# Hagtaril/HiddenPose

Hardware: AMD Instinct MI355X
Metric: samples/sec (128x128x512 meas) fwd+bwd (higher is better)
Workload: dtype f32; 1 GPU; NlosPose train step (fwd+L2Joint+BCEDice loss+bwd+Adam), 128x128x512 transients, batch 4/GPU, fp32, random-init weights, weight gradients of the 3^3 / 4^3 convolutions (and of small 1^3 ones) on a second stream; global_batch=4, world_size=1, parallelism=dp1

## Files before the change

hiddenpose_amd/csrc/conv_kernels.hip:

```cpp
#include <algorithm>
#include <cstdlib>
#include <cstring>
#include <mutex>
#include <type_traits>
#include <vector>

#include "hp_internal.h"

namespace hp {

using f32x16 = __attribute__((ext_vector_type(16))) float;
using bf16x8 = __attribute__((ext_vector_type(8))) __bf16;
using bf16x4 = __attribute__((ext_vector_type(4))) __bf16;
using bf16x2 = __attribute__((ext_vector_type(2))) __bf16;
using f32x2 = __attribute__((ext_vector_type(2))) float;
using s16x4 = __attribute__((ext_vector_type(4))) short;

__device__ __forceinline__ bf16x4 to_bf16x4(const float4 v) {
  const bf16x2 lo = __builtin_convertvector((f32x2){v.x, v.y}, bf16x2);
  const bf16x2 hi = __builtin_convertvector((f32x2){v.z, v.w}, bf16x2);
  return (bf16x4){lo[0], lo[1], hi[0], hi[1]};
}

enum IgemmMode { MODE_CONV = 0, MODE_DECONV = 1, MODE_DGRAD_S2K3 = 2, MODE_STEM = 3 };
// ... 2016 lines not shown
    for (int i = 0; i < 2; ++i)
#pragma unroll
      for (int r = 0; r < 16; ++r) {
        const int co = i * 32 + (r & 3) + 8 * (r >> 2) + 4 * half;
        if (tap < 343) atomicAdd(dW + (long)co * kpad + tap, acc[i][j][r]);
      }
  }
}

constexpr int SFH_TZ = 16, SFH_TY = 4, SFH_TX = 8, SFH_PZ = SFH_TZ + 6, SFH_PR = 28, SFH_PP = 10 * SFH_PR;
constexpr int SFH_COPY = SFH_PZ * SFH_PP + 8;
constexpr int SFH_W = 50 * 64 * 8;
constexpr int SFH_NP = SFH_PZ * 10 * 14;
constexpr int SFH_LD = (SFH_NP + 511) / 512;

__global__ __launch_bounds__(512) void k_stem_fwd_bf16(const float* __restrict__ X, const float* __restrict__ Wp,
                                                       float* __restrict__ Y, double* __restrict__ stats, int D, int H, int W,
                                                       int kpad, int pz, int py, int px, long tiles_total, int tiles_per_wg) {
  extern __shared__ __attribute__((aligned(16))) float sfh_smem[];
  __bf16* const wl = (__bf16*)sfh_smem;
  __bf16* const patch = wl + SFH_W;
  float* const red = (float*)(patch + 4 * SFH_COPY);
  const int tid = threadIdx.x, lane = tid & 63, wave = tid >> 6, col = lane & 31, half = lane >> 5;
  for (int sidx = tid; sidx < 50 * 64; sidx += 512) {
    const int pr = sidx >> 6, n = sidx & 63;
    float v[8];
#pragma unroll
    for (int c = 0; c < 8; ++c) v[c] = (pr < 49 && c < 7) ? Wp[(long)n * kpad + pr * 7 + c] : 0.f;
    *(bf16x4*)(wl + sidx * 8) = to_bf16x4(make_float4(v[0], v[1], v[2], v[3]));
    *(bf16x4*)(wl + sidx * 8 + 4) = to_bf16x4(make_float4(v[4], v[5], v[6], v[7]));
  }
  for (int i = tid; i < 4 * SFH_COPY / 2; i += 512) ((unsigned int*)patch)[i] = 0u;
  const long t0 = (long)blockIdx.x * tiles_per_wg, t1 = min(tiles_total, t0 + tiles_per_wg);
  float preg[SFH_LD];
  auto tile_origin = [&](long t, int& b, int& z0, int& y0, int& x0) {
    long r_ = t;
    x0 = (int)(r_ % px) * SFH_TX;
    r_ /= px;
    y0 = (int)(r_ % py) * SFH_TY;
    r_ /= py;
    z0 = (int)(r_ % pz) * SFH_TZ;
    b = (int)(r_ / pz);
  };
  auto fetch = [&](long t) {
    int b, z0, y0, x0;
    tile_origin(t, b, z0, y0, x0);
#pragma unroll
    for (int k = 0; k < SFH_LD; ++k) {
      const int e = tid + 512 * k;
      const int pzz = e / 140, rem = e - pzz * 140, pyy = rem / 14, pxx = rem - pyy * 14;
      const int z = z0 + pzz - 3, y = y0 + pyy - 3, x = x0 + pxx - 3;
      preg[k] = (e < SFH_NP && (unsigned)z < (unsigned)D && (unsigned)y < (unsigned)H && (unsigned)x < (unsigned)W)
                    ? X[(((long)b * D + z) * H + y) * W + x]
                    : 0.f;
    }
  };
  int abase[2];
#pragma unroll
  for (int mt = 0; mt < 2; ++mt) abase[mt] = (2 * wave + mt) * SFH_PP + (col >> 3) * SFH_PR + (col & 7);
  float ssum[2] = {0.f, 0.f}, ssq[2] = {0.f, 0.f};
  if (t0 < t1) fetch(t0);
  for (long t = t0; t < t1; ++t) {
    __syncthreads();
#pragma unroll
    for (int k = 0; k < SFH_LD; ++k) {
      const int e = tid + 512 * k;
      const int pzz = e / 140, rem = e - pzz * 140, pyy = rem / 14, pxx = rem - pyy * 14;
      if (e < SFH_NP) {
        const int pi = pzz * SFH_PP + pyy * SFH_PR + pxx;
        const __bf16 v = (__bf16)preg[k];
#pragma unroll
        for (int sft = 0; sft < 4; ++sft)
          if (pi - sft >= 0) patch[sft * SFH_COPY + pi - sft] = v;
      }
    }
    __syncthreads();
    int b, z0, y0, x0;
    tile_origin(t, b, z0, y0, x0);
    if (t + 1 < t1) fetch(t + 1);
    f32x16 acc[2][2];
#pragma unroll
    for (int mt = 0; mt < 2; ++mt)
#pragma unroll
      for (int nt = 0; nt < 2; ++nt)
#pragma unroll
        for (int r = 0; r < 16; ++r) acc[mt][nt][r] = 0.f;
    int kd = 0, kh = half;
#pragma unroll 5
    for (int ks = 0; ks < 25; ++ks) {
      const int pr = 2 * ks + half;
      const int off = pr < 49 ? kd * SFH_PP + kh * SFH_PR : 0;
      bf16x8 ha[2], hb[2];
#pragma unroll
      for (int mt = 0; mt < 2; ++mt) {
        const int e = abase[mt] + off;
        const __bf16* const src = patch + (e & 3) * SFH_COPY + (e & ~3);
        union {
          uint2 q[2];
          bf16x8 f;
        } u;
        u.q[0] = *(const uint2*)(src);
        u.q[1] = *(const uint2*)(src + 4);
        ha[mt] = u.f;
      }
#pragma unroll
      for (int nt = 0; nt < 2; ++nt) hb[nt] = *(const bf16x8*)(wl + ((pr * 64) + nt * 32 + col) * 8);
#pragma unroll
      for (int mt = 0; mt < 2; ++mt)
#pragma unroll
        for (int nt = 0; nt < 2; ++nt) acc[mt][nt] = __builtin_amdgcn_mfma_f32_32x32x16_bf16(ha[mt], hb[nt], acc[mt][nt], 0, 0, 0);
      kh += 2;
      if (kh >= 7) {
        kh -= 7;
        ++kd;
      }
    }
#pragma unroll
    for (int mt = 0; mt < 2; ++mt) {
      const int z = z0 + 2 * wave + mt;
#pragma unroll
      for (int r = 0; r < 16; ++r) {
        const int i = (r & 3) + 8 * (r >> 2) + 4 * half;
        const int y = y0 + (i >> 3), x = x0 + (i & 7);
        if (z < D && y < H && x < W) {
          float* const yo = Y + ((((long)b * D + z) * H + y) * W + x) * 64 + col;
#pragma unroll
          for (int nt = 0; nt < 2; ++nt) {
            const float v = acc[mt][nt][r];
            yo[nt * 32] = v;
            ssum[nt] += v;
            ssq[nt] += v * v;
          }
        }
      }
    }
  }
  if (stats) {
#pragma unroll
    for (int nt = 0; nt < 2; ++nt) {
      const float sv = ssum[nt] + __shfl_xor(ssum[nt], 32), qv = ssq[nt] + __shfl_xor(ssq[nt], 32);
      if (half == 0) {
        red[(wave * 64 + nt * 32 + col) * 2 + 0] = sv;
        red[(wave * 64 + nt * 32 + col) * 2 + 1] = qv;
      }
    }
    __syncthreads();
    if (tid < 64) {
      double sv = 0.0, qv = 0.0;
#pragma unroll
      for (int w = 0; w < 8; ++w) {
        sv += (double)red[(w * 64 + tid) * 2 + 0];
        qv += (double)red[(w * 64 + tid) * 2 + 1];
      }
      double* const slot = stats + (size_t)(blockIdx.x & (HP_STATS_SLOTS - 1)) * 128;
      atomicAdd(slot + tid, sv);
      atomicAdd(slot + 64 + tid, qv);
    }
  }
}

constexpr int SF_TY = 8, SF_TX = 64, SF_RY = SF_TY + 6, SF_RX = 72, SF_PLANE = SF_RY * SF_RX;
using f32x4c = __attribute__((ext_vector_type(4))) float;

__global__ __launch_bounds__(256) void k_stem_fwd_mfma(const float* __restrict__ X, const float* __restrict__ Wp,
                                                       float* __restrict__ Y, double* __restrict__ stats, int D, int H, int W,
                                                       int kpad, int tiles_x, int tiles_y, int zchunk) {
  extern __shared__ __attribute__((aligned(16))) float sf_smem[];
  float* const wl = sf_smem;
  float* const ring = wl + 343 * 64;
  float* const otile = ring + 8 * SF_PLANE;
  const int tid = threadIdx.x, lane = tid & 63, wave = tid >> 6, sub = lane & 3;
  int t_ = blockIdx.x;
  const int bx = t_ % tiles_x;
  t_ /= tiles_x;
  const int by = t_ % tiles_y;
  const int bz = t_ / tiles_y;
  const int b = blockIdx.y;
  const int x0 = bx * SF_TX, y0 = by * SF_TY;
  const int zb = bz * zchunk, ze = min(D, zb + zchunk);
  const float* xb = X + (long)b * D * H * W;

  for (int e = tid; e < 343 * 64; e += 256) {
    const int cg = e & 15, i = (e >> 4) & 3, tap = e >> 6;
    wl[e] = Wp[(long)(cg * 4 + i) * kpad + tap];
  }
  constexpr int SK = (SF_PLANE + 255) / 256;
  int soff[SK];
  unsigned smask = 0;
#pragma unroll
  for (int k = 0; k < SK; ++k) {
    const int e = tid + 256 * k;
    const int ly = e / SF_RX, lx = e - ly * SF_RX;
    const int yy = y0 + ly - 3, xx = x0 + lx - 3;
    const bool ok = e < SF_PLANE && lx < SF_TX + 6 && (unsigned)yy < (unsigned)H && (unsigned)xx < (unsigned)W;
    soff[k] = ok ? yy * W + xx : 0;
    smask |= ok ? (1u << k) : 0u;
  }
  auto stage_load = [&](int zin, float (&v)[SK]) {
    const bool zok = (unsigned)zin < (unsigned)D;
    const float* src = xb + (long)(zok ? zin : 0) * H * W;
#pragma unroll
    for (int k = 0; k < SK; ++k) v[k] = (zok && ((smask >> k) & 1u)) ? src[soff[k]] : 0.f;
  };
  auto stage_store = [&](int zin, const float (&v)[SK]) {
    float* dst = ring + (zin & 7) * SF_PLANE + tid;
#pragma unroll
    for (int k = 0; k < SK; ++k)
      if (tid + 256 * k < SF_PLANE) dst[256 * k] = v[k];
  };
  auto stage = [&](int zin) {
    float v[SK];
    stage_load(zin, v);
    stage_store(zin, v);
  };
  if (zb < ze)
    for (int zin = zb - 3; zin <= zb + 3; ++zin) stage(zin);
  __syncthreads();

  float* const ot = otile + wave * (64 * 33);
  float ssum[2] = {0.f, 0.f}, ssq[2] = {0.f, 0.f};
  for (int z = zb; z < ze; ++z) {
    float nv[SK];
    if (z + 1 < ze) stage_load(z + 4, nv);
    __builtin_amdgcn_sched_barrier(0);
    f32x4c acc[2][16];
#pragma unroll
    for (int r = 0; r < 2; ++r)
#pragma unroll
      for (int cg = 0; cg < 16; ++cg) acc[r][cg] = (f32x4c){0.f, 0.f, 0.f, 0.f};
#pragma unroll 1
    for (int a = 0; a < 7; ++a) {
      const float* pl = ring + ((z + a - 3) & 7) * SF_PLANE + (2 * wave) * SF_RX + lane;
#pragma unroll
      for (int bb = 0; bb < 7; ++bb) {
        const float* wt = wl + ((a * 7 + bb) * 7) * 64 + sub * 16;
#pragma unroll
        for (int c = 0; c < 7; ++c) {
          float wr[16];
#pragma unroll
          for (int q = 0; q < 4; ++q) {
            const f32x4c t4 = *(const f32x4c*)(wt + c * 64 + 4 * q);
            wr[4 * q] = t4[0];
            wr[4 * q + 1] = t4[1];
            wr[4 * q + 2] = t4[2];
            wr[4 * q + 3] = t4[3];
          }
#pragma unroll
          for (int r = 0; r < 2; ++r) {
            const float xv = pl[(r + bb) * SF_RX + c];
#pragma unroll
            for (int cg = 0; cg < 16; ++cg) acc[r][cg] = __builtin_amdgcn_mfma_f32_4x4x1f32(wr[cg], xv, acc[r][cg], 0, 0, 0);
          }
        }
      }
    }
#pragma unroll
    for (int r = 0; r < 2; ++r) {
      const int oy = y0 + 2 * wave + r;
      const bool row_ok = oy < H;
      const long orow = (((long)b * D + z) * H + oy) * W + x0;
#pragma unroll
      for (int hh = 0; hh < 2; ++hh) {
#pragma unroll
        for (int cg = 0; cg < 8; ++cg)
#pragma unroll
          for (int i = 0; i < 4; ++i) ot[lane * 33 + cg * 4 + i] = acc[r][8 * hh + cg][i];
        if (row_ok) {
          if (stats && lane < 32) {
            float s = 0.f, q = 0.f;
            const int nv = min(64, W - x0);
            for (int v = 0; v < nv; ++v) {
              const float val = ot[v * 33 + lane];
              s += val;
              q += val * val;
            }
            ssum[hh] += s;
            ssq[hh] += q;
          }
          const int q4 = lane & 7;
#pragma unroll
          for (int it = 0; it < 8; ++it) {
            const int v = it * 8 + (lane >> 3);
            if (x0 + v < W) {
              const float* sp = ot + v * 33 + 4 * q4;
              *(float4*)(Y + (orow + v) * 64 + 32 * hh + 4 * q4) = make_float4(sp[0], sp[1], sp[2], sp[3]);
            }
          }
        }
      }
    }
    if (z + 1 < ze) stage_store(z + 4, nv);
    __syncthreads();
  }
  if (stats && lane < 32) {
#pragma unroll
    for (int hh = 0; hh < 2; ++hh) {
      double* const slot = stats + (size_t)(blockIdx.x & (HP_STATS_SLOTS - 1)) * 128;
      atomicAdd(slot + 32 * hh + lane, (double)ssum[hh]);
      atomicAdd(slot + 64 + 32 * hh + lane, (double)ssq[hh]);
    }
  }
}

__global__ void k_pack_weight(const float* __restrict__ w, float* __restrict__ out, int Cout, int Cin, int taps,
                              int transposed, int swap, int to_torch) {
  const long total = (long)Cout * Cin * taps;
  for (long i = (long)blockIdx.x * blockDim.x + threadIdx.x; i < total; i += (long)gridDim.x * blockDim.x) {
    const int inner = (int)(i % (swap ? Cout : Cin));
    long r = i / (swap ? Cout : Cin);
    const int outer = (int)(r % (swap ? Cin : Cout));
    const int t = (int)(r / (swap ? Cin : Cout));
    const int co = swap ? inner : outer, ci = swap ? outer : inner;
    const long ti = transposed ? ((long)ci * Cout + co) * taps + t : ((long)co * Cin + ci) * taps + t;
    if (to_torch)
      ((float*)w)[ti] = out[i];
    else
      out[i] = w[ti];
  }
}

__global__ __launch_bounds__(256) void k_pack_weight_tiled(const float* __restrict__ w, float* __restrict__ out, int Cout,
                                                           int Cin, int taps, int transposed, int swap, int to_torch,
                                                           int out_half = 0) {
  __shared__ float tile[64][65];
  const int A = swap ? Cin : Cout, Bn = swap ? Cout : Cin;
  const int a = blockIdx.y, bn0 = blockIdx.x * 64;
  const int nb = min(64, Bn - bn0), n = nb * taps;
  auto torch_index = [&](int bn, int t) -> long {
    const int co = swap ? bn : a, ci = swap ? a : bn;
    return transposed ? ((long)ci * Cout + co) * taps + t : ((long)co * Cin + ci) * taps + t;
  };
  if (!to_torch) {
    for (int e = threadIdx.x; e < n; e += 256) {
      const int bl = e / taps, t = e - bl * taps;
      tile[bl][t] = w[torch_index(bn0 + bl, t)];
    }
    __syncthreads();
    for (int e = threadIdx.x; e < taps * 64; e += 256) {
      const int t = e >> 6, bl = e & 63;
      if (bl < nb) hp_st1(out, ((long)t * A + a) * Bn + bn0 + bl, tile[bl][t], out_half);
    }
  } else {
    for (int e = threadIdx.x; e < taps * 64; e += 256) {
      const int t = e >> 6, bl = e & 63;
      if (bl < nb) tile[bl][t] = out[((long)t * A + a) * Bn + bn0 + bl];
    }
    __syncthreads();
    for (int e = threadIdx.x; e < n; e += 256) {
      const int bl = e / taps, t = e - bl * taps;
      ((float*)w)[torch_index(bn0 + bl, t)] = tile[bl][t];
    }
  }
}

__global__ void k_pack_stem(const float* __restrict__ w, float* __restrict__ out, int Cout, int kpad, int to_torch) {
  const long total = (long)Cout * kpad;
  for (long i = (long)blockIdx.x * blockDim.x + threadIdx.x; i < total; i += (long)gridDim.x * blockDim.x) {
    const int k = (int)(i % kpad), n = (int)(i / kpad);
    if (to_torch) {
      if (k < 343) ((float*)w)[(long)n * 343 + k] = out[i];
    } else {
      out[i] = k < 343 ? w[(long)n * 343 + k] : 0.f;
    }
  }
}

struct ConvPlan {
  IgemmGeom fwd, dgrad, wgrad;
  int fwd_classes = 1, dgrad_classes = 1, wgrad_tapsum = 1;
  bool stem = false, dgrad_zero_fill = false;
  int planes = 0;
};

static void set_shifts(IgemmGeom& g) {
  g.sw = g.sh = g.sd = -1;
  if (g.mode >= 0 && is_pow2(g.gw) && is_pow2(g.gh) && is_pow2(g.gd) && g.M < (1l << 32)) {
    g.sw = ilog2(g.gw);
    g.sh = ilog2(g.gh);
    g.sd = ilog2(g.gd);
  }
}

static int make_plan(const hp_conv_desc& d, ConvPlan& p) {
  HP_REQUIRE(d.B >= 1 && d.Cin >= 1 && d.Cout >= 1, "conv: bad channel/batch sizes");
  HP_REQUIRE(d.precision >= HP_PRECISION_FP32 && d.precision <= HP_PRECISION_BF16X6, "conv: unknown precision %d", d.precision);
  HP_REQUIRE(d.io == 0 || d.precision == HP_PRECISION_BF16, "conv: bf16 activation tensors (io = %d) go with HP_PRECISION_BF16", d.io);
  p.planes = d.precision;
  const int k = d.k, s = d.stride, pad = d.pad;
  IgemmGeom f{};
  if (!d.transposed) {
    const int Do = (d.Di + 2 * pad - k) / s + 1, Ho = (d.Hi + 2 * pad - k) / s + 1, Wo = (d.Wi + 2 * pad - k) / s + 1;
    p.stem = (d.Cin == 1 && k == 7 && s == 1 && pad == 3);
    if (!p.stem) HP_REQUIRE(d.Cin % 4 == 0, "conv: Cin must be a multiple of 4 (got %d)", d.Cin);
    HP_REQUIRE(s == 1 || s == 2, "conv: stride must be 1 or 2");
    const int kpt = p.stem ? (343 + 31) / 32 : (d.Cin + 31) / 32;
    f = IgemmGeom{p.stem ? MODE_STEM : MODE_CONV, d.B, d.Di, d.Hi, d.Wi, d.Cin, Do, Ho, Wo, d.Cout, Do, Ho, Wo, 1,
                  k, s, pad, 0, (long)d.B * Do * Ho * Wo, kpt};
    p.fwd = f;
    p.fwd_classes = 1;
    p.wgrad = f;
    p.wgrad_tapsum = p.stem ? 1 : k * k * k;
    IgemmGeom g{};
    if (p.stem) {
      g = IgemmGeom{MODE_CONV, d.B, Do, Ho, Wo, d.Cout, d.Di, d.Hi, d.Wi, 1, d.Di, d.Hi, d.Wi, 1,
                    7, 1, 3, 1, (long)d.B * d.Di * d.Hi * d.Wi, d.Cout / 32};
      p.dgrad_classes = 1;
    } else if (s == 1) {
      HP_REQUIRE(d.Cout % 4 == 0, "conv dgrad: Cout must be a multiple of 4 (got %d)", d.Cout);
      g = IgemmGeom{MODE_CONV, d.B, Do, Ho, Wo, d.Cout, d.Di, d.Hi, d.Wi, d.Cin, d.Di, d.Hi, d.Wi, 1,
                    k, 1, pad, 1, (long)d.B * d.Di * d.Hi * d.Wi, (d.Cout + 31) / 32};
      p.dgrad_classes = 1;
    } else if (k == 3 && pad == 1) {
      HP_REQUIRE(d.Di % 2 == 0 && d.Hi % 2 == 0 && d.Wi % 2 == 0 && d.Cout % 32 == 0, "conv dgrad s2: even dims needed");
      g = IgemmGeom{MODE_DGRAD_S2K3, d.B, Do, Ho, Wo, d.Cout, d.Di, d.Hi, d.Wi, d.Cin, d.Di / 2, d.Hi / 2, d.Wi / 2, 2,
                    3, 1, 1, 0, (long)d.B * (d.Di / 2) * (d.Hi / 2) * (d.Wi / 2), d.Cout / 32};
      p.dgrad_classes = 8;
    } else if (k == 1 && pad == 0) {
      HP_REQUIRE(d.Di % 2 == 0 && d.Hi % 2 == 0 && d.Wi % 2 == 0 && d.Cout % 32 == 0, "conv dgrad s2: even dims needed");
      g = IgemmGeom{MODE_CONV, d.B, Do, Ho, Wo, d.Cout, d.Di, d.Hi, d.Wi, d.Cin, Do, Ho, Wo, 2,
                    1, 1, 0, 0, (long)d.B * Do * Ho * Wo, d.Cout / 32};
      p.dgrad_classes = 1;
      p.dgrad_zero_fill = true;
    } else {
      set_error("conv: unsupported stride-2 kernel %d pad %d", k, pad);
      return HP_ERR_UNSUPPORTED;
    }
    p.dgrad = g;
  } else {
    HP_REQUIRE(k == 4 && s == 2 && pad == 1, "deconv: only k4 s2 p1 is supported");
    HP_REQUIRE(d.Cin % 32 == 0 && d.Cout % 32 == 0, "deconv: channels must be multiples of 32");
    const int Do = 2 * d.Di, Ho = 2 * d.Hi, Wo = 2 * d.Wi;
    f = IgemmGeom{MODE_DECONV, d.B, d.Di, d.Hi, d.Wi, d.Cin, Do, Ho, Wo, d.Cout, d.Di, d.Hi, d.Wi, 2,
                  4, 1, 1, 0, (long)d.B * d.Di * d.Hi * d.Wi, d.Cin / 32};
    p.fwd = f;
    p.fwd_classes = 8;
    p.wgrad = f;
    p.wgrad_tapsum = 64;
    p.dgrad = IgemmGeom{MODE_CONV, d.B, Do, Ho, Wo, d.Cout, d.Di, d.Hi, d.Wi, d.Cin, d.Di, d.Hi, d.Wi, 1,
                        4, 2, 1, 0, (long)d.B * d.Di * d.Hi * d.Wi, d.Cout / 32};
    p.dgrad_classes = 1;
  }
  HP_REQUIRE((long)d.B * d.Di * d.Hi * d.Wi * (d.transposed ? 8 : 1) < (1l << 31), "conv: more than 2^31 voxels per tensor");
  set_shifts(p.fwd);
  set_shifts(p.dgrad);
  set_shifts(p.wgrad);
  p.fwd.welems = p.wgrad.welems = p.stem ? (long)d.Cout * ((343 + 31) / 32 * 32) : (long)d.Cout * d.Cin * k * k * k;
  p.dgrad.welems = (long)d.Cout * d.Cin * k * k * k;
  return HP_OK;
}

template <bool STEM, bool STATS, int NP, bool XH = false>
static void launch_igemm_bn(const IgemmGeom& g, int classes, const void* X, const float* W, const float* bias, void* Y,
                            double* stats, const void* addend, const unsigned char* amask, hipStream_t st) {
  if constexpr (NP == 1 && !STEM && !XH) {
    if (g.xh && g.Cin % 64 == 0) return launch_igemm_bn<STEM, STATS, NP, true>(g, classes, X, W, bias, Y, stats, addend, amask, st);
  }
  const unsigned mt = (unsigned)((g.M + BM - 1) / BM);
  static const bool gl_on = !(getenv("HP_IGEMM_GL") && atoi(getenv("HP_IGEMM_GL")) == 0);
  const bool gl = XH && g.wh && gl_on;
  static const bool bl_on = !(getenv("HP_IGEMM_BL") && atoi(getenv("HP_IGEMM_BL")) == 0);
  const bool bl = !XH && !g.xh && !g.wh && !STEM && bl_on && g.Cin % 32 == 0 && (long)g.Nout * g.Cin * class_ntaps(g, 0) * 4 * (g.mode == MODE_DECONV ? 8 : 1) < (1l << 31);
  static const bool slab_on = !(getenv("HP_IGEMM_SLAB") && atoi(getenv("HP_IGEMM_SLAB")) == 0);
  if (slab_on && g.Nout <= 64) {
    IgemmGeom gs = g;
    gs.slab = (int)((mt + 7) / 8);
    const dim3 grid((mt + 7) / 8 * 8, 1, classes);
    if constexpr (!XH && !STEM) {
      if (bl && g.Nout > 32) {
        hipLaunchKernelGGL((k_igemm<64, false, STATS, NP, false, false, true>), grid, dim3(CT), 0, st, X, W, bias, Y, stats, addend, amask, gs);
        return;
      }
    }
  }
  if (g.Nout > 64) {
    const unsigned tn = (unsigned)((g.Nout + 127) / 128);
    IgemmGeom gg = g;
    gg.tn = tn > 1 ? (int)tn : 0;
    gg.slab = slab_on ? (int)((mt + 7) / 8) : 0;
    const dim3 grid = (tn > 1 || gg.slab) ? dim3((mt + 7) / 8 * 8 * (tn > 1 ? tn : 1), 1, classes) : dim3(mt, 1, classes);
    if constexpr (XH) {
      if (gl) {
        hipLaunchKernelGGL((k_igemm<128, STEM, STATS, NP, true, true>), grid, dim3(CT), 0, st, X, W, bias, Y, stats, addend, amask, gg);
        return;
      }
    }
    if constexpr (!XH && !STEM) {
      if (bl) {
        hipLaunchKernelGGL((k_igemm<128, false, STATS, NP, false, false, true>), grid, dim3(CT), 0, st, X, W, bias, Y, stats, addend, amask, gg);
        return;
      }
    }
    hipLaunchKernelGGL((k_igemm<128, STEM, STATS, NP, XH>), grid, dim3(CT), 0, st, X, W, bias, Y, stats, addend, amask, gg);
  } else if (g.Nout > 32) {
    if constexpr (XH) {
      if (gl) {
        hipLaunchKernelGGL((k_igemm<64, STEM, STATS, NP, true, true>), dim3(mt, 1, classes), dim3(CT), 0, st, X, W, bias, Y, stats, addend, amask, g);
        return;
      }
    }
    if constexpr (!XH && !STEM) {
      if (bl) {
        hipLaunchKernelGGL((k_igemm<64, false, STATS, NP, false, false, true>), dim3(mt, 1, classes), dim3(CT), 0, st, X, W, bias, Y, stats, addend, amask, g);
        return;
      }
    }
    hipLaunchKernelGGL((k_igemm<64, STEM, STATS, NP, XH>), dim3(mt, 1, classes), dim3(CT), 0, st, X, W, bias, Y, stats, addend, amask, g);
  } else {
    hipLaunchKernelGGL((k_igemm<32, STEM, STATS, NP, XH>), dim3(mt, 1, classes), dim3(CT), 0, st, X, W, bias, Y, stats, addend, amask, g);
  }
}

template <int NP>
static void launch_igemm_p(const IgemmGeom& g, int classes, bool stem, const void* X, const float* W, const float* bias,
                           void* Y, double* stats, const void* addend, const unsigned char* amask, hipStream_t st) {
  if (stem) {
    if (stats) launch_igemm_bn<true, true, NP>(g, classes, X, W, bias, Y, stats, addend, amask, st);
    else launch_igemm_bn<true, false, NP>(g, classes, X, W, bias, Y, stats, addend, amask, st);
  } else {
    if (stats) launch_igemm_bn<false, true, NP>(g, classes, X, W, bias, Y, stats, addend, amask, st);
    else launch_igemm_bn<false, false, NP>(g, classes, X, W, bias, Y, stats, addend, amask, st);
  }
}

static void launch_igemm(const IgemmGeom& g, int classes, bool stem, int planes, const void* X, const float* W,
                         const float* bias, void* Y, double* stats, const void* addend, hipStream_t st,
                         const unsigned char* amask = nullptr) {
  switch (planes) {
    case 1: launch_igemm_p<1>(g, classes, stem, X, W, bias, Y, stats, addend, amask, st); break;
    case 2: launch_igemm_p<2>(g, classes, stem, X, W, bias, Y, stats, addend, amask, st); break;
    case 3: launch_igemm_p<3>(g, classes, stem, X, W, bias, Y, stats, addend, amask, st); break;
    default: launch_igemm_p<0>(g, classes, stem, X, W, bias, Y, stats, addend, amask, st); break;
  }
}

}

using namespace hp;

extern "C" size_t hp_conv3d_packed_weight_elems(const hp_conv_desc* d) {
  if (!d) return 0;
  if (!d->transposed && d->Cin == 1 && d->k == 7) return (size_t)d->Cout * ((343 + 31) / 32 * 32);
  return (size_t)d->Cout * d->Cin * d->k * d->k * d->k;
}

extern "C" int hp_conv3d_pack_weight(const hp_conv_desc* d, const float* w_torch, void* w_fwd_v, void* w_dgrad_v,
                                     void* stream) {
  float* const w_fwd = (float*)w_fwd_v;
  float* const w_dgrad = (float*)w_dgrad_v;
  HP_REQUIRE(d && w_torch, "hp_conv3d_pack_weight: null argument");
  ConvPlan p;
  int rc = make_plan(*d, p);
  if (rc) return rc;
  hipStream_t st = (hipStream_t)stream;
  const int taps = d->k * d->k * d->k;
  if (p.stem) {
    const int kpad = p.fwd.kpt * BK;
    HP_PROF("conv_pack_weight", st);
    if (w_fwd) hipLaunchKernelGGL(k_pack_stem, dim3(64), dim3(256), 0, st, w_torch, w_fwd, d->Cout, kpad, 0);
    if (w_dgrad) hipLaunchKernelGGL(k_pack_weight, dim3(64), dim3(256), 0, st, w_torch, w_dgrad, d->Cout, 1, 343, 0, 1, 0);
  } else {
    HP_REQUIRE(taps <= 64, "conv: at most 64 taps (got %d)", taps);
    HP_PROF("conv_pack_weight", st);
    const int wh = (d->io & HP_IO_W_BF16) ? 1 : 0;
    if (w_fwd)
      hipLaunchKernelGGL(k_pack_weight_tiled, dim3((d->Cin + 63) / 64, d->Cout), dim3(256), 0, st, w_torch, w_fwd, d->Cout,
                         d->Cin, taps, d->transposed, 0, 0, wh);
    if (w_dgrad)
      hipLaunchKernelGGL(k_pack_weight_tiled, dim3((d->Cout + 63) / 64, d->Cin), dim3(256), 0, st, w_torch, w_dgrad, d->Cout,
                         d->Cin, taps, d->transposed, 1, 0, wh);
  }
  HP_CHECK_HIP(hipGetLastError());
  return HP_OK;
}

extern "C" int hp_conv3d_unpack_wgrad(const hp_conv_desc* d, const float* dw_packed, float* dw_torch, void* stream) {
  HP_REQUIRE(d && dw_packed && dw_torch, "hp_conv3d_unpack_wgrad: null argument");
  ConvPlan p;
  int rc = make_plan(*d, p);
  if (rc) return rc;
  hipStream_t st = (hipStream_t)stream;
  const int taps = d->k * d->k * d->k;
  HP_PROF("conv_pack_weight", st);
  if (p.stem) {
    hipLaunchKernelGGL(k_pack_stem, dim3(64), dim3(256), 0, st, dw_torch, (float*)dw_packed, d->Cout, p.fwd.kpt * BK, 1);
  } else {
    hipLaunchKernelGGL(k_pack_weight_tiled, dim3((d->Cin + 63) / 64, d->Cout), dim3(256), 0, st, dw_torch, (float*)dw_packed,
                       d->Cout, d->Cin, taps, d->transposed, 0, 1);
  }
  HP_CHECK_HIP(hipGetLastError());
  return HP_OK;
}

extern "C" int hp_conv3d_forward(const hp_conv_desc* d, const void* x, const float* w_fwd, const float* bias, void* y,
                                 double* stats, void* stream) {
  HP_REQUIRE(d && x && w_fwd && y, "hp_conv3d_forward: null argument");
  ConvPlan p;
  int rc = make_plan(*d, p);
  if (rc) return rc;
  HP_REQUIRE(!(p.stem && (d->io & HP_IO_X_BF16)), "hp_conv3d_forward: the stem reads its single-channel input as fp32");
  p.fwd.xh = (d->io & HP_IO_X_BF16) ? 1 : 0;
  p.fwd.yh = (d->io & HP_IO_Y_BF16) ? 1 : 0;
  p.fwd.wh = (d->io & HP_IO_W_BF16) ? 1 : 0;
  HP_REQUIRE(!p.fwd.wh || (p.fwd.xh && p.planes == 1 && !p.stem && d->Cin % 64 == 0),
             "hp_conv3d_forward: bf16 packed weights go with a bf16 input, HP_PRECISION_BF16 and Cin %% 64 == 0");
  hipStream_t st = (hipStream_t)stream;
  if (stats) HP_CHECK_HIP(hipMemsetAsync(stats, 0, sizeof(double) * 2 * d->Cout * HP_STATS_SLOTS, st));
  if (p.stem && p.planes == 1 && d->Cout == 64 && !bias && !p.fwd.yh) {
    const int pz = (d->Di + SFH_TZ - 1) / SFH_TZ, py = (d->Hi + SFH_TY - 1) / SFH_TY, px = (d->Wi + SFH_TX - 1) / SFH_TX;
    const long tiles = (long)d->B * pz * py * px;
    const int per_wg = (int)std::max<long>(1, (tiles + 511) / 512);
    const size_t lds = sizeof(__bf16) * (SFH_W + 4 * SFH_COPY) + sizeof(float) * 8 * 64 * 2;
    static std::once_flag lds_once_h;
    static hipError_t lds_rc_h = hipSuccess;
    std::call_once(lds_once_h, [&] {
      lds_rc_h = hipFuncSetAttribute((const void*)k_stem_fwd_bf16, hipFuncAttributeMaxDynamicSharedMemorySize, (int)lds);
    });
    HP_CHECK_HIP(lds_rc_h);
    HP_PROF("conv_igemm_stem", st);
    hipLaunchKernelGGL(k_stem_fwd_bf16, dim3((unsigned)((tiles + per_wg - 1) / per_wg)), dim3(512), lds, st, (const float*)x, w_fwd,
                       (float*)y, stats, d->Di, d->Hi, d->Wi, p.fwd.kpt * BK, pz, py, px, tiles, per_wg);
  } else if (p.stem && p.planes == 0 && d->Cout == 64 && !bias && !p.fwd.yh) {
    const int tiles_x = (d->Wi + SF_TX - 1) / SF_TX, tiles_y = (d->Hi + SF_TY - 1) / SF_TY;
    const long cols = (long)tiles_x * tiles_y * d->B;
    int zsplit = (int)std::max<long>(1, std::min<long>((d->Di + 15) / 16, (1024 + cols - 1) / cols));
    const int zchunk = (d->Di + zsplit - 1) / zsplit;
    zsplit = (d->Di + zchunk - 1) / zchunk;
    const size_t lds = sizeof(float) * (343 * 64 + 8 * SF_PLANE + 4 * 64 * 33);
    static std::once_flag lds_once;
    static hipError_t lds_rc = hipSuccess;
    std::call_once(lds_once, [&] {
      lds_rc = hipFuncSetAttribute((const void*)k_stem_fwd_mfma, hipFuncAttributeMaxDynamicSharedMemorySize, (int)lds);
    });
    HP_CHECK_HIP(lds_rc);
    HP_PROF("conv_igemm_stem", st);
    hipLaunchKernelGGL(k_stem_fwd_mfma, dim3((unsigned)(tiles_x * tiles_y * zsplit), (unsigned)d->B), dim3(256), lds, st,
                       (const float*)x, w_fwd, (float*)y, stats, d->Di, d->Hi, d->Wi, p.fwd.kpt * BK, tiles_x, tiles_y, zchunk);
  } else {
    HP_PROF(p.stem ? "conv_igemm_stem" : d->transposed ? "conv_igemm_deconv" : d->k == 1 ? "conv_igemm_k1" : "conv_igemm_k3", st);
    launch_igemm(p.fwd, p.fwd_classes, p.stem, p.planes, x, w_fwd, bias, y, stats, nullptr, st);
  }
  HP_CHECK_HIP(hipGetLastError());
  return HP_OK;
}

extern "C" int hp_linear_forward(const float* x, const float* w, const float* bias, const float* addend, float* y, long M, int K,
                                 int N, int precision, void* stream) {
  HP_REQUIRE(x && w && y && M >= 1 && M < (1l << 31) && K >= 4 && N >= 1, "hp_linear_forward: bad argument");
  hp_conv_desc d{1, 1, 1, (int)M, K, N, 1, 1, 0, 0, precision, 0};
  ConvPlan p;
  int rc = make_plan(d, p);
  if (rc) return rc;
  hipStream_t st = (hipStream_t)stream;
  {
    HP_PROF("linear_fwd", st);
    launch_igemm(p.fwd, 1, false, p.planes, x, w, bias, y, nullptr, addend, st);
  }
  HP_CHECK_HIP(hipGetLastError());
  return HP_OK;
}

extern "C" int hp_linear_geglu_forward(const float* x, const float* w, const float* bias, float* y, long M, int K,
                                       int N2, int precision, void* stream) {
  HP_REQUIRE(x && w && y && M >= 1 && M < (1l << 31) && K >= 4, "hp_linear_geglu_forward: bad argument");
  HP_REQUIRE(N2 >= 128 && N2 % 128 == 0, "hp_linear_geglu_forward: 2 * hidden must be a multiple of 128 (got %d)", N2);
  hp_conv_desc d{1, 1, 1, (int)M, K, N2, 1, 1, 0, 0, precision, 0};
  ConvPlan p;
  int rc = make_plan(d, p);
  if (rc) return rc;
  p.fwd.geglu = 1;
  hipStream_t st = (hipStream_t)stream;
  {
    HP_PROF("linear_fwd", st);
    launch_igemm(p.fwd, 1, false, p.planes, x, w, bias, y, nullptr, nullptr, st);
  }
  HP_CHECK_HIP(hipGetLastError());
  return HP_OK;
}

static bool launch_igemm_bns(const IgemmGeom& g, const void* X, const float* W, void* Y, const void* addend,
                             const unsigned char* amask, hipStream_t st) {
  const bool dense_out = g.os == 1 && g.gd == g.Do && g.gh == g.Ho && g.gw == g.Wo;
  if (g.mode != MODE_CONV || !dense_out || g.M % BM != 0 || g.Nout <= 32 || g.Nout % (g.Nout > 64 ? 128 : 64) != 0 || g.xh || g.yh ||
      g.wh || g.ah)
    return false;
  const unsigned mt = (unsigned)(g.M / BM);
  static const bool bl_on = !(getenv("HP_IGEMM_BL") && atoi(getenv("HP_IGEMM_BL")) == 0);
  static const bool slab_on = !(getenv("HP_IGEMM_SLAB") && atoi(getenv("HP_IGEMM_SLAB")) == 0);
  const bool bl = bl_on && g.Cin % 32 == 0 && (long)g.Nout * g.Cin * class_ntaps(g, 0) * 4 < (1l << 31);
  IgemmGeom gg = g;
  gg.slab = slab_on ? (int)((mt + 7) / 8) : 0;
#define HP_BNS_LAUNCH(BN_, BL_)                                                                                                     \
  do {                                                                                                                             \
    if (g.bn_mask)                                                                                                                 \
      hipLaunchKernelGGL((k_igemm<BN_, false, false, 0, false, false, BL_, 2>), grid, dim3(CT), 0, st, X, W, nullptr, Y, nullptr,   \
                         addend, amask, gg);                                                                                       \
    else                                                                                                                           \
      hipLaunchKernelGGL((k_igemm<BN_, false, false, 0, false, false, BL_, 1>), grid, dim3(CT), 0, st, X, W, nullptr, Y, nullptr,   \
                         addend, amask, gg);                                                                                       \
  } while (0)
  if (g.Nout <= 64) {
    const dim3 grid = gg.slab ? dim3((mt + 7) / 8 * 8, 1, 1) : dim3(mt, 1, 1);
    if (bl) HP_BNS_LAUNCH(64, true);
    else HP_BNS_LAUNCH(64, false);
    return true;
  }
  const unsigned tn = (unsigned)(g.Nout / 128);
  gg.tn = tn > 1 ? (int)tn : 0;
  const dim3 grid = (tn > 1 || gg.slab) ? dim3((mt + 7) / 8 * 8 * (tn > 1 ? tn : 1), 1, 1) : dim3(mt, 1, 1);
  if (bl) HP_BNS_LAUNCH(128, true);
  else HP_BNS_LAUNCH(128, false);
#undef HP_BNS_LAUNCH
  return true;
}

extern "C" int hp_conv3d_backward_data_bnsums(const hp_conv_desc* d, const void* dy, const float* w_dgrad, void* dx, const void* addend,
                                              const unsigned char* addend_mask, const float* z, const float* mean,
                                              const float* rstd, const float* gamma, const float* beta, int relu,
                                              const unsigned char* relu_mask, double* sums, int* fused, void* stream) {
  HP_REQUIRE(d && dy && w_dgrad && dx && z && mean && rstd && sums && fused && (!relu || relu_mask || (gamma && beta)),
             "hp_conv3d_backward_data_bnsums: null argument");
  *fused = 0;
  ConvPlan p;
  int rc = make_plan(*d, p);
  if (rc) return rc;
  hipStream_t st = (hipStream_t)stream;
  if (p.planes == 0 && !p.stem && !p.dgrad_zero_fill && d->io == 0 && p.dgrad_classes == 1 &&
      (!addend_mask || (addend && d->Cin % 4 == 0 && d->Cin > 32))) {
    IgemmGeom g = p.dgrad;
    g.bn_z = z;
    g.bn_mean = mean;
    g.bn_rstd = rstd;
    g.bn_gamma = gamma;
    g.bn_beta = beta;
    g.bn_sums = sums;
    g.bn_relu = relu ? 1 : 0;
    g.bn_mask = relu ? relu_mask : nullptr;
    HP_CHECK_HIP(hipMemsetAsync(sums, 0, sizeof(double) * 2 * g.Nout * HP_STATS_SLOTS, st));
    HP_PROF("conv_igemm_dgrad", st);
    if (launch_igemm_bns(g, dy, w_dgrad, dx, addend, addend_mask, st)) {
      HP_CHECK_HIP(hipGetLastError());
      *fused = 1;
      return HP_OK;
    }
  }
  return hp_conv3d_backward_data_masked(d, dy, w_dgrad, dx, addend, addend_mask, stream);
}

extern "C" int hp_conv3d_backward_data(const hp_conv_desc* d, const void* dy, const float* w_dgrad, void* dx,
                                       const void* addend, void* stream) {
  return hp_conv3d_backward_data_masked(d, dy, w_dgrad, dx, addend, nullptr, stream);
}

extern "C" int hp_conv3d_backward_data_masked(const hp_conv_desc* d, const void* dy, const float* w_dgrad, void* dx,
                                              const void* addend, const unsigned char* addend_mask, void* stream) {
  HP_REQUIRE(d && dy && w_dgrad && dx, "hp_conv3d_backward_data: null argument");
  ConvPlan p;
  int rc = make_plan(*d, p);
  if (rc) return rc;
  const int dyh = (d->io & HP_IO_DY_BF16) ? 1 : 0, dxh = (d->io & HP_IO_DX_BF16) ? 1 : 0;
  HP_REQUIRE(!(p.stem && (dyh || dxh)), "hp_conv3d_backward_data: the stem's data gradient is fp32 in, fp32 out");
  p.dgrad.xh = dyh;
  p.dgrad.yh = p.dgrad.ah = dxh;
  p.dgrad.wh = (d->io & HP_IO_W_BF16) ? 1 : 0;
  HP_REQUIRE(!p.dgrad.wh || (dyh && p.planes == 1 && !p.stem && p.dgrad.Cin % 64 == 0),
             "hp_conv3d_backward_data: bf16 packed weights go with a bf16 dy, HP_PRECISION_BF16 and Cout %% 64 == 0");
  const size_t esz = dxh ? 2 : 4;
  HP_REQUIRE(!addend_mask || (addend && !p.stem && !p.dgrad_zero_fill && d->Cin % 4 == 0 && d->Cin > 32),
             "hp_conv3d_backward_data_masked: a masked addend needs a dense data gradient with > 32 input channels, a multiple of 4");
  hipStream_t st = (hipStream_t)stream;
  if (p.stem) {
    HP_REQUIRE(d->Cout == 64, "stem data gradient: 64 output channels expected (got %d)", d->Cout);
    HP_REQUIRE((long)d->Hi * d->Wi <= (1l << 21), "stem data gradient: H * W up to 2^21 (31-bit offsets inside a 4-plane dZ tile), got %d x %d", d->Hi, d->Wi);
    const size_t nb = sizeof(float) * (size_t)d->B * d->Di * d->Hi * d->Wi;
    if (addend) HP_CHECK_HIP(hipMemcpyAsync(dx, addend, nb, hipMemcpyDeviceToDevice, st));
    else HP_CHECK_HIP(hipMemsetAsync(dx, 0, nb, st));
    const int pz = (d->Di + SP_Z - 1) / SP_Z, py = (d->Hi + SP_Y - 1) / SP_Y, px = (d->Wi + SP_X - 1) / SP_X;
    HP_PROF("conv_stem_dgrad", st);
    const long cols = (long)py * px * d->B;
    int zsplit = 1;
    long best = -1;
    for (int zs = 1; zs <= std::min(pz, 32); ++zs) {
      const long cost = ((cols * zs + 767) / 768) * ((pz + zs - 1) / zs + 2);
      if (best < 0 || cost < best) best = cost, zsplit = zs;
    }
    if (const char* e = getenv("HP_STEM_DGRAD_ZSPLIT")) zsplit = std::max(1, std::min(pz, atoi(e)));
    const int zchunk = (pz + zsplit - 1) / zsplit;
    zsplit = (pz + zchunk - 1) / zchunk;
    hipLaunchKernelGGL(p.planes == 1 ? k_stem_dgrad<true> : k_stem_dgrad<false>, dim3((unsigned)(py * px * zsplit), (unsigned)d->B), dim3(CT), 0,
                       st, (const float*)dy, w_dgrad, (float*)dx, d->Di, d->Hi, d->Wi, pz, py, px, zchunk);
    HP_CHECK_HIP(hipGetLastError());
    return HP_OK;
  }
  if (p.dgrad_zero_fill) {
    const size_t nb = esz * (size_t)d->B * d->Di * d->Hi * d->Wi * d->Cin;
    if (addend == dx) {}
    else if (addend) HP_CHECK_HIP(hipMemcpyAsync(dx, addend, nb, hipMemcpyDeviceToDevice, st));
    else HP_CHECK_HIP(hipMemsetAsync(dx, 0, nb, st));
  }
  {
    HP_PROF("conv_igemm_dgrad", st);
    launch_igemm(p.dgrad, p.dgrad_classes, false, p.planes, dy, w_dgrad, nullptr, dx, nullptr, addend, st, addend_mask);
  }
  HP_CHECK_HIP(hipGetLastError());
  return HP_OK;
}

struct WgradSplit {
  int TT, tap_groups, tiles_c, tiles_total;
  bool multitap;
  long msplit;
};
static WgradSplit wgrad_split(const ConvPlan& p) {
  const IgemmGeom& g = p.wgrad;
  const int Kc = p.stem ? g.kpt * BK : g.Cin;
  WgradSplit w{};
  w.TT = (g.Nout >= 128 && Kc >= 128) ? 128 : 64;
  w.multitap = !p.stem && w.TT == 64 && g.mode == MODE_CONV && g.k == 3;
  w.tap_groups = w.multitap ? (27 + 3) / 4 : p.wgrad_tapsum;
  const int tiles_n = (g.Nout + w.TT - 1) / w.TT;
  w.tiles_c = (Kc + w.TT - 1) / w.TT;
  const long base_blocks = (long)tiles_n * w.tiles_c * w.tap_groups;
  long hi = std::max<long>(1, (4096 + base_blocks - 1) / base_blocks);
  hi = std::min<long>(std::min<long>(hi, std::max<long>(1, g.M / (4 * WG_KM))), 4096);
  static const int fixed_env = getenv("HP_WGRAD_R0") ? atoi(getenv("HP_WGRAD_R0")) : -1;
  const long r0 = fixed_env >= 0 ? fixed_env : ((g.xh && g.yh) ? 768 : 96);
  long best = hi;
  struct Memo { long M, base, r0, hi, best; };
  static std::mutex memo_mu;
  static std::vector<Memo> memo;
  bool known = false;
  {
    std::lock_guard<std::mutex> lk(memo_mu);
    for (const Memo& m : memo)
      if (m.M == g.M && m.base == base_blocks && m.r0 == r0 && m.hi == hi) {
        best = m.best;
        known = true;
        break;
      }
  }
  if (r0 > 0 && !known) {
    const long slots = 768;
    auto cost = [&](long ms) {
      const long rows = ((g.M + ms - 1) / ms + WG_KM - 1) / WG_KM * WG_KM;
      const long blocks = base_blocks * ms;
      double c = (double)((blocks + slots - 1) / slots) * (double)(rows + r0);
      if (blocks & 7) c *= 1.02;
      return c;
    };
    double cmin = cost(hi);
    for (long ms = 1; ms < hi; ++ms) cmin = std::min(cmin, cost(ms));
    for (long ms = hi; ms >= 1; --ms)
      if (cost(ms) <= 1.03 * cmin) {
        best = ms;
        break;
      }
  }
  for (; !known;) {
    const long chunk = ((g.M + best - 1) / best + WG_KM - 1) / WG_KM * WG_KM;
    const long need = (g.M + chunk - 1) / chunk;
    if (need >= best) break;
    best = need;
  }
  if (!known) {
    std::lock_guard<std::mutex> lk(memo_mu);
    if (memo.size() < 4096) memo.push_back({g.M, base_blocks, r0, hi, best});
  }
  w.msplit = best;
  w.tiles_total = tiles_n * w.tiles_c;
  return w;
}

extern "C" int hp_conv3d_backward_weight_split(const hp_conv_desc* d, long* msplit, long* chunk_rows) {
  HP_REQUIRE(d && msplit && chunk_rows, "hp_conv3d_backward_weight_split: null argument");
  ConvPlan p;
  int rc = make_plan(*d, p);
  if (rc) return rc;
  p.wgrad.xh = (d->io & HP_IO_X_BF16) ? 1 : 0;
  p.wgrad.yh = (d->io & HP_IO_DY_BF16) ? 1 : 0;
  const WgradSplit ws = wgrad_split(p);
  *msplit = ws.msplit;
  *chunk_rows = ((p.wgrad.M + ws.msplit - 1) / ws.msplit + WG_KM - 1) / WG_KM * WG_KM;
  return HP_OK;
}

extern "C" int hp_conv3d_backward_weight(const hp_conv_desc* d, const void* x, const void* dy, float* dw_packed,
                                         void* stream) {
  HP_REQUIRE(d && x && dy && dw_packed, "hp_conv3d_backward_weight: null argument");
  ConvPlan p;
  int rc = make_plan(*d, p);
  if (rc) return rc;
  hipStream_t st = (hipStream_t)stream;
  const int xh = (d->io & HP_IO_X_BF16) ? 1 : 0, dyh = (d->io & HP_IO_DY_BF16) ? 1 : 0;
  HP_REQUIRE(!(p.stem && xh), "hp_conv3d_backward_weight: the stem reads its single-channel input as fp32");
  p.wgrad.xh = xh;
  p.wgrad.yh = dyh;
  const IgemmGeom& g = p.wgrad;
  const int Kc = p.stem ? g.kpt * BK : g.Cin;
  HP_CHECK_HIP(hipMemsetAsync(dw_packed, 0, sizeof(float) * hp_conv3d_packed_weight_elems(d), st));
  if (p.stem && p.planes <= 1 && d->Cout == 64 && !dyh) {
    const int pz = (d->Di + SP_Z - 1) / SP_Z, py = (d->Hi + SP_Y - 1) / SP_Y, px = (d->Wi + SP_X - 1) / SP_X;
    const long tiles = (long)d->B * pz * py * px;
    const int per_wg = (int)std::max<long>(1, (tiles + 1023) / 1024);
    HP_PROF("conv_wgrad", st);
    hipLaunchKernelGGL(p.planes == 1 ? k_stem_wgrad_bf16 : k_stem_wgrad_full, dim3((unsigned)((tiles + per_wg - 1) / per_wg)), dim3(256),
                       0, st, (const float*)x, (const float*)dy, dw_packed, d->Di,
                       d->Hi, d->Wi, pz, py, px, tiles, per_wg, Kc);
    HP_CHECK_HIP(hipGetLastError());
    return HP_OK;
  }
  if (!p.stem && p.planes == 0 && !xh && !dyh && g.mode == MODE_CONV && g.k == 1 && g.s == 1 && g.os == 1 && g.M >= (1l << 16)) {
    const bool wide_n = g.Nout % 256 == 0 && g.Cin == 64, wide_c = g.Nout == 64 && g.Cin % 256 == 0;
    if (wide_n || wide_c) {
      const int tiles = wide_n ? g.Nout / 256 : g.Cin / 256;
      long ms = std::max<long>(1, std::min<long>(1024 / tiles, g.M / (4 * WG_KM)));
      ms = std::max<long>(8, ms / 8 * 8);
      HP_PROF("conv_wgrad", st);
      if (wide_n)
        hipLaunchKernelGGL((k_wgrad_dense<256, 64>), dim3((unsigned)(tiles * ms)), dim3(CT), 0, st, (const float*)x, (const float*)dy, dw_packed, g.M, g.Nout,
                           g.Cin, (int)ms, 1);
      else
        hipLaunchKernelGGL((k_wgrad_dense<64, 256>), dim3((unsigned)(tiles * ms)), dim3(CT), 0, st, (const float*)x, (const float*)dy, dw_packed, g.M, g.Nout,
                           g.Cin, (int)ms, tiles);
      HP_CHECK_HIP(hipGetLastError());
      return HP_OK;
    }
  }
  const WgradSplit ws = wgrad_split(p);
  const int TT = ws.TT, tap_groups = ws.tap_groups, tiles_c = ws.tiles_c, tiles_total = ws.tiles_total;
  const bool multitap = ws.multitap;
  const long msplit = ws.msplit;
  dim3 grid((unsigned)((long)tiles_total * tap_groups * msplit));
  {
    HP_PROF("conv_wgrad", st);
    static const bool wbl_on = !(getenv("HP_WGRAD_BL") && atoi(getenv("HP_WGRAD_BL")) == 0);
    const long chunk_rows = (g.M + msplit - 1) / msplit + WG_KM;
    const long span_y = chunk_rows * g.os * g.os * g.os * (long)g.Nout * 4, span_x = (chunk_rows * g.s * g.s * g.s + 4l * g.Hi * g.Wi) * (long)g.Cin * 4;
    const bool exact_grid = g.Di == g.gd * g.s && g.Hi == g.gh * g.s && g.Wi == g.gw * g.s && g.Do == g.gd * g.os &&
                            g.Ho == g.gh * g.os && g.Wo == g.gw * g.os;
    if (wbl_on && !p.stem && p.planes == 0 && !xh && !dyh && g.sw >= 0 && exact_grid && g.Nout % 4 == 0 && g.Cin % 4 == 0 &&
// ... 70 lines not shown
```

Before: 8.783 samples/s.

## Add fp32 stem forward kernel using 32x32x2 MFMA with explicit LDS pipelining

Adds a new stem convolution forward kernel (7^3 taps, Cin=1, Cout=64) built on mfma_f32_32x32x2f32 in place of the older 4x4x1-based route. It pairs taps per MFMA step, issues LDS reads through inline asm with immediate offsets, and double-buffers fragments under explicit waitcnt and sched barriers. BN statistics are reduced in LDS before one atomic per channel. The old kernel stays reachable through an environment variable. This costs extra LDS and register pressure and depends on hand-written asm ordering.

```diff
diff --git a/hiddenpose_amd/csrc/conv_kernels.hip b/hiddenpose_amd/csrc/conv_kernels.hip
--- a/hiddenpose_amd/csrc/conv_kernels.hip
+++ b/hiddenpose_amd/csrc/conv_kernels.hip
@@ -2342,6 +2342,196 @@
   }
 }
 
+constexpr int SF32_WL = 344 * 64;
+constexpr int SF32_ZP = 160;
+
+__device__ __forceinline__ unsigned lds_addr(const float* p) {
+  return (unsigned)(size_t)(const __attribute__((address_space(3))) float*)p;
+}
+
+template <int S, int N, class F>
+__device__ __forceinline__ void static_for(F&& f) {
+  if constexpr (S < N) {
+    f(std::integral_constant<int, S>{});
+    static_for<S + 1, N>(f);
+  }
+}
+
+__global__ __launch_bounds__(256) void k_stem_fwd_mfma32(const float* __restrict__ X, const float* __restrict__ Wp,
+                                                         float* __restrict__ Y, double* __restrict__ stats, int D, int H, int W,
+                                                         int kpad, int tiles_x, int tiles_y, int zchunk) {
+  extern __shared__ __attribute__((aligned(16))) float sf_smem[];
+  float* const wl = sf_smem;
+  float* const ring = wl + SF32_WL;
+  float* const red = ring + 8 * SF_PLANE;
+  float* const zpad = red + 8 * 128;
+  const int tid = threadIdx.x, lane = tid & 63, wave = tid >> 6, col = lane & 31, half = lane >> 5;
+  int t_ = blockIdx.x;
+  const int bx = t_ % tiles_x;
+  t_ /= tiles_x;
+  const int by = t_ % tiles_y;
+  const int bz = t_ / tiles_y;
+  const int b = blockIdx.y;
+  const int x0 = bx * SF_TX, y0 = by * SF_TY;
+  const int zb = bz * zchunk, ze = min(D, zb + zchunk);
+  const float* xb = X + (long)b * D * H * W;
+
+  for (int e = tid; e < SF32_WL; e += 256) {
+    const int n = e & 63, tap = e >> 6;
+    wl[e] = tap < 343 ? Wp[(long)n * kpad + tap] : 0.f;
+  }
+  if (tid < SF32_ZP) zpad[tid] = 0.f;
+  constexpr int SK = (SF_PLANE + 255) / 256;
+  int soff[SK];
+  unsigned smask = 0;
+#pragma unroll
+  for (int k = 0; k < SK; ++k) {
+    const int e = tid + 256 * k;
+    const int ly = e / SF_RX, lx = e - ly * SF_RX;
+    const int yy = y0 + ly - 3, xx = x0 + lx - 3;
+    const bool ok = e < SF_PLANE && lx < SF_TX + 6 && (unsigned)yy < (unsigned)H && (unsigned)xx < (unsigned)W;
+    soff[k] = ok ? yy * W + xx : 0;
+    smask |= ok ? (1u << k) : 0u;
+  }
+  auto stage_load = [&](int zin, float (&v)[SK]) {
+    const bool zok = (unsigned)zin < (unsigned)D;
+    const float* src = xb + (long)(zok ? zin : 0) * H * W;
+#pragma unroll
+    for (int k = 0; k < SK; ++k) v[k] = (zok && ((smask >> k) & 1u)) ? src[soff[k]] : 0.f;
+  };
+  auto stage_store = [&](int zin, const float (&v)[SK]) {
+    float* dst = ring + (zin & 7) * SF_PLANE + tid;
+#pragma unroll
+    for (int k = 0; k < SK; ++k)
+      if (tid + 256 * k < SF_PLANE) dst[256 * k] = v[k];
+  };
+  if (zb < ze)
+    for (int zin = zb - 3; zin <= zb + 3; ++zin) {
+      float v[SK];
+      stage_load(zin, v);
+      stage_store(zin, v);
+    }
+  __syncthreads();
+
+  const unsigned wb0 = lds_addr(wl + half * 64 + col);
+  const unsigned wb1 = wb0 + 4u * 128 * 128;
+  const unsigned lanebase = lds_addr(ring + (2 * wave) * SF_RX + col);
+  const unsigned zbase = lds_addr(zpad + col) - 4u * (6 * SF_RX + 6);
+  const bool full_x = x0 + SF_TX <= W;
+  float ssum[2] = {0.f, 0.f}, ssq[2] = {0.f, 0.f};
+  for (int z = zb; z < ze; ++z) {
+    float nv[SK];
+    if (z + 1 < ze) stage_load(z + 4, nv);
+    unsigned pp[7], pq[7], ps[3], pl;
+#pragma unroll
+    for (int kd = 0; kd < 7; ++kd) {
+      const unsigned pb = lanebase + 4u * (unsigned)(((z + kd - 3) & 7) * SF_PLANE);
+      pp[kd] = pb + 4u * half;
+      pq[kd] = pb + 4u * 66 * half;
+    }
+#pragma unroll
+    for (int i = 0; i < 3; ++i)
+      ps[i] = lanebase + 4u * (unsigned)(half ? ((z + 2 * i - 2) & 7) * SF_PLANE : ((z + 2 * i - 3) & 7) * SF_PLANE + 6 * SF_RX + 6);
+    pl = half ? zbase : lanebase + 4u * (unsigned)(((z + 3) & 7) * SF_PLANE);
+    __builtin_amdgcn_sched_barrier(0);
+    f32x16 acc[2][2][2];
+#pragma unroll
+    for (int r = 0; r < 2; ++r)
+#pragma unroll
+      for (int xh = 0; xh < 2; ++xh)
+#pragma unroll
+        for (int j = 0; j < 2; ++j)
+#pragma unroll
+          for (int q = 0; q < 16; ++q) acc[r][xh][j][q] = 0.f;
+    float fa[2][4], fb[2][2];
+    auto frag = [&](auto sc, float (&a)[4], float (&w)[2]) {
+      constexpr int s = decltype(sc)::value, te = 2 * s, to = 2 * s + 1;
+      constexpr int kde = te / 49, khe = (te / 7) % 7, kwe = te % 7;
+      constexpr int kdo = to / 49, kho = (to / 7) % 7;
+      constexpr int imm = 4 * ((to != 343 && kdo != kde) ? 0 : khe * SF_RX + kwe);
+      const unsigned base = to == 343 ? pl : kdo != kde ? ps[kde >> 1] : kho != khe ? pq[kde] : pp[kde];
+      asm volatile("ds_read_b32 %0, %1 offset:%2" : "=v"(a[0]) : "v"(base), "n"(imm));
+      asm volatile("ds_read_b32 %0, %1 offset:%2" : "=v"(a[1]) : "v"(base), "n"(imm + 4 * 32));
+      asm volatile("ds_read_b32 %0, %1 offset:%2" : "=v"(a[2]) : "v"(base), "n"(imm + 4 * SF_RX));
+      asm volatile("ds_read_b32 %0, %1 offset:%2" : "=v"(a[3]) : "v"(base), "n"(imm + 4 * (SF_RX + 32)));
+      constexpr int wimm = 4 * 128 * (s < 128 ? s : s - 128);
+      const unsigned wbs = s < 128 ? wb0 : wb1;
+      asm volatile("ds_read_b32 %0, %1 offset:%2" : "=v"(w[0]) : "v"(wbs), "n"(wimm));
+      asm volatile("ds_read_b32 %0, %1 offset:%2" : "=v"(w[1]) : "v"(wbs), "n"(wimm + 4 * 32));
+    };
+    auto arrive = [&](float (&a)[4], float (&w)[2]) {
+      asm volatile("s_waitcnt lgkmcnt(0)" : "+v"(a[0]), "+v"(a[1]), "+v"(a[2]), "+v"(a[3]), "+v"(w[0]), "+v"(w[1])::"memory");
+    };
+    frag(std::integral_constant<int, 0>{}, fa[0], fb[0]);
+    arrive(fa[0], fb[0]);
+    static_for<0, 172>([&](auto sc) {
+      constexpr int s = decltype(sc)::value;
+      if constexpr (s + 1 < 172) frag(std::integral_constant<int, s + 1>{}, fa[(s + 1) & 1], fb[(s + 1) & 1]);
+      __builtin_amdgcn_sched_barrier(0);
+#pragma unroll
+      for (int r = 0; r < 2; ++r)
+#pragma unroll
+        for (int xh = 0; xh < 2; ++xh)
+#pragma unroll
+          for (int j = 0; j < 2; ++j)
+            acc[r][xh][j] = __builtin_amdgcn_mfma_f32_32x32x2f32(fa[s & 1][2 * r + xh], fb[s & 1][j], acc[r][xh][j], 0, 0, 0);
+      __builtin_amdgcn_sched_barrier(0);
+      if constexpr (s + 1 < 172) arrive(fa[(s + 1) & 1], fb[(s + 1) & 1]);
+      __builtin_amdgcn_sched_barrier(0);
+    });
+    float sl[2] = {0.f, 0.f}, ql[2] = {0.f, 0.f};
+    auto emit = [&](auto full) {
+#pragma unroll
+      for (int r = 0; r < 2; ++r) {
+        const int oy = y0 + 2 * wave + r;
+        if (oy >= H) continue;
+        float* const yrow = Y + ((((long)b * D + z) * H + oy) * W + x0) * 64;
+#pragma unroll
+        for (int xh = 0; xh < 2; ++xh)
+#pragma unroll
+          for (int q = 0; q < 16; ++q) {
+            const int m = 32 * xh + (q & 3) + 8 * (q >> 2) + 4 * half;
+            if (decltype(full)::value || x0 + m < W) {
+#pragma unroll
+              for (int j = 0; j < 2; ++j) {
+                const float v = acc[r][xh][j][q];
+                yrow[m * 64 + 32 * j + col] = v;
+                sl[j] += v;
+                ql[j] += v * v;
+              }
+            }
+          }
+      }
+    };
+    if (full_x)
+      emit(std::true_type{});
+    else
+      emit(std::false_type{});
+#pragma unroll
+    for (int j = 0; j < 2; ++j) {
+      ssum[j] += sl[j];
+      ssq[j] += ql[j];
+    }
+    if (z + 1 < ze) stage_store(z + 4, nv);
+    __syncthreads();
+  }
+  if (stats) {
+#pragma unroll
+    for (int j = 0; j < 2; ++j) {
+      red[((wave * 2 + half) * 2 + 0) * 64 + 32 * j + col] = ssum[j];
+      red[((wave * 2 + half) * 2 + 1) * 64 + 32 * j + col] = ssq[j];
+    }
+    __syncthreads();
+    if (tid < 128) {
+      double v = 0.0;
+#pragma unroll
+      for (int k = 0; k < 8; ++k) v += (double)red[k * 128 + tid];
+      double* const slot = stats + (size_t)(blockIdx.x & (HP_STATS_SLOTS - 1)) * 128;
+      atomicAdd(slot + tid, v);
+    }
+  }
+}
+
 __global__ void k_pack_weight(const float* __restrict__ w, float* __restrict__ out, int Cout, int Cin, int taps,
                               int transposed, int swap, int to_torch) {
   const long total = (long)Cout * Cin * taps;
@@ -2666,15 +2856,24 @@
     const int zchunk = (d->Di + zsplit - 1) / zsplit;
     zsplit = (d->Di + zchunk - 1) / zchunk;
     const size_t lds = sizeof(float) * (343 * 64 + 8 * SF_PLANE + 4 * 64 * 33);
+    const size_t lds32 = sizeof(float) * (SF32_WL + 8 * SF_PLANE + 8 * 128 + SF32_ZP);
     static std::once_flag lds_once;
     static hipError_t lds_rc = hipSuccess;
     std::call_once(lds_once, [&] {
       lds_rc = hipFuncSetAttribute((const void*)k_stem_fwd_mfma, hipFuncAttributeMaxDynamicSharedMemorySize, (int)lds);
+      if (lds_rc == hipSuccess)
+        lds_rc = hipFuncSetAttribute((const void*)k_stem_fwd_mfma32, hipFuncAttributeMaxDynamicSharedMemorySize, (int)lds32);
     });
     HP_CHECK_HIP(lds_rc);
+    const char* const route = getenv("HP_STEM_FWD");
+    const bool old_route = route && !strcmp(route, "4x4x1");
     HP_PROF("conv_igemm_stem", st);
-    hipLaunchKernelGGL(k_stem_fwd_mfma, dim3((unsigned)(tiles_x * tiles_y * zsplit), (unsigned)d->B), dim3(256), lds, st,
-                       (const float*)x, w_fwd, (float*)y, stats, d->Di, d->Hi, d->Wi, p.fwd.kpt * BK, tiles_x, tiles_y, zchunk);
+    if (old_route)
+      hipLaunchKernelGGL(k_stem_fwd_mfma, dim3((unsigned)(tiles_x * tiles_y * zsplit), (unsigned)d->B), dim3(256), lds, st,
+                         (const float*)x, w_fwd, (float*)y, stats, d->Di, d->Hi, d->Wi, p.fwd.kpt * BK, tiles_x, tiles_y, zchunk);
+    else
+      hipLaunchKernelGGL(k_stem_fwd_mfma32, dim3((unsigned)(tiles_x * tiles_y * zsplit), (unsigned)d->B), dim3(256), lds32, st,
+                         (const float*)x, w_fwd, (float*)y, stats, d->Di, d->Hi, d->Wi, p.fwd.kpt * BK, tiles_x, tiles_y, zchunk);
   } else {
     HP_PROF(p.stem ? "conv_igemm_stem" : d->transposed ? "conv_igemm_deconv" : d->k == 1 ? "conv_igemm_k1" : "conv_igemm_k3", st);
     launch_igemm(p.fwd, p.fwd_classes, p.stem, p.planes, x, w_fwd, bias, y, stats, nullptr, st);
```

Result: no change. 8.830 samples/s, median of 6 (+0.5%).
